# scrose/SVDSolver

Hardware: AMD Instinct MI355X
Metric: GFLOP/s for two-stage bidiag reduction, N×N fp64, 1/2/4/8 MI355X (higher is better)
Workload: dtype f64; 1 GPU; stream of independent two-stage bidiagonal reductions 8192x8192 f64, band 32, stage 2 = reference window geometry (compat); n=8192, band=32, global_batch=10, parallelism=replicas1, pipeline=stage 2 of matrix i on a second HIP stream beside stage 1 of matrix i+1, stage2_cus=32, lanes=10, stage2_streams=5, hw_queues=19

## Files before the change

svdsolver_amd/csrc/brd_blk.h:

```cpp
#pragma once

#include "brd_internal.h"

#include <hip/hip_ext.h>

#include <climits>

namespace brd {
namespace blk {

template <typename T> struct Mf;
template <> struct Mf<double> {
    typedef double v4 __attribute__((ext_vector_type(4)));
    static __device__ __forceinline__ v4 mma(double a, double b, v4 c) {
        return __builtin_amdgcn_mfma_f64_16x16x4f64(a, b, c, 0, 0, 0);
    }
    static __device__ __forceinline__ int crow(int q, int g) { return q + 4 * g; }
};
template <> struct Mf<float> {
    typedef float v4 __attribute__((ext_vector_type(4)));
    static __device__ __forceinline__ v4 mma(float a, float b, v4 c) {
        return __builtin_amdgcn_mfma_f32_16x16x4f32(a, b, c, 0, 0, 0);
    }
    static __device__ __forceinline__ int crow(int q, int g) { return 4 * q + g; }
// ... 11 lines not shown
constexpr int kWM = 64;
constexpr int kMT = 256;
#ifndef BRD_BLK_KSU
#define BRD_BLK_KSU 8
#endif
constexpr int kSU = BRD_BLK_KSU;

constexpr int kRpLds = 8192;
struct RpArgs {
    const void *src;  long ld;
    const void *vsrc; long vld;
    const void *bsrc; long bld;
    int K, M;
    int mtiles, ksplit, kper;
    int tiles, ns, wst;
    int nvirt;
    void *part; long mp;
    void *vpart;
    void *vout;
    int *counter;
    int *err;
    int has_fin;
    int vfold = 0;
    int va = 0, vb = 0;
};

constexpr int kPT = 256;
constexpr int kPI = 32;

constexpr int kGramRec = 1040;
struct PrepArgs {
    void *A; long lda;
    void *Lw; void *RwT; long ldr;
    const void *part; long mp; int ksplit;
    const void *G;
    const void *Tm;
    void *Qp;
    long mq;
    int c;
    int j;
    int items;
    int reduce, factor;
    const double *sgn;
    int split;
    long cc;
    int zfill;
// ... 286 lines not shown
template <typename T, int AUX = 0> __device__ __forceinline__ T buf_ld(__amdgpu_buffer_rsrc_t r, unsigned off) {
    if constexpr (sizeof(T) == 8)
        return __builtin_bit_cast(double, __builtin_amdgcn_raw_buffer_load_b64(r, (int)off, 0, AUX));
    else
        return __builtin_bit_cast(float, __builtin_amdgcn_raw_buffer_load_b32(r, (int)off, 0, AUX));
}
template <typename T, int AUX = 0> __device__ __forceinline__ void buf_st(T v, __amdgpu_buffer_rsrc_t r, unsigned off) {
    if constexpr (sizeof(T) == 8)
        __builtin_amdgcn_raw_buffer_store_b64(__builtin_bit_cast(u32x2_t, v), r, (int)off, 0, AUX);
    else
        __builtin_amdgcn_raw_buffer_store_b32(__builtin_bit_cast(unsigned, v), r, (int)off, 0, AUX);
}

template <typename F, typename... Args>
static inline void blk_launch(const char *kind, double flops, double bytes, F kernel, dim3 grid, dim3 block,
                              hipStream_t s, Args... args) {
    hipEvent_t ea, eb;
    if (api_prof_launch_events(kind, flops, bytes, &ea, &eb, (int)(grid.x * grid.y)))
        hipExtLaunchKernelGGL(kernel, grid, block, 0, s, ea, eb, 0, args...);
    else
        hipLaunchKernelGGL(kernel, grid, block, 0, s, args...);
}

bool rpass_dma_ok(bool yp, int K, int M, size_t elem, const void *src, long ld, const void *vsrc, long vld,
                  const void *bsrc, long bld);
int rpass_stage_k(size_t elem);
template <typename T>
void launch_k_rpass(bool yp, dim3 grid, const RpArgs &a, const FinArgs &f, hipStream_t s, double fl, double by);
template <typename T>
void launch_k_vsum(const T *vpart, T *vout, int nvirt, T *pbase, long pstride, const double *sgn, hipStream_t s);
template <typename T>
void launch_k_prep(bool lq, dim3 grid, const PrepArgs &p, hipStream_t s);
enum CqrKernel { kCqrGram, kCqrQ1, kCqrV, kCqrVInline, kCqrMid };
template <typename T>
void launch_k_cqr(CqrKernel which, int nwg, const CqrArgs &a, const FinArgs &f, hipStream_t s);
template <typename T>
void launch_k_blkupd(dim3 grid, const GemmArgs &g, hipStream_t s, double fl, double by);
template <typename T>
void launch_dist_unpack_v(const T *src, T *dst, int M, hipStream_t s);
template <typename T>
void launch_dist_psum(const T *part, int ks, long mp, int rows, T *buf, hipStream_t s);

}
}
```

svdsolver_amd/csrc/brd_blk_prep.hip:

```cpp
#include "brd_blk.h"

#include <climits>
#include <cstdlib>

namespace brd {
namespace blk {


#ifndef BRD_GRAM_LSCOPE
#define BRD_GRAM_LSCOPE __HIP_MEMORY_SCOPE_AGENT
#endif
#ifndef BRD_GRAM_SSCOPE
#define BRD_GRAM_SSCOPE __HIP_MEMORY_SCOPE_AGENT
#endif
template <typename FILL>
__device__ __forceinline__ void prep_gram(const PrepArgs &a, int nwv, int wv, int ipw, double *tile, double *red,
                                          double *smax, int *sflag, FILL &&fill) {
    typedef Mf<double>::v4 v4d;
    const int lane = threadIdx.x & 63, q = lane >> 4, l15 = lane & 15;
    const int nt = 64 * nwv, tl = 64 * wv + lane;
    __syncthreads();
    double *tw = tile + wv * 16 * 33;
    fill(tw);
    __builtin_amdgcn_fence(__ATOMIC_RELEASE, "wavefront");
// ... 498 lines not shown
    __builtin_amdgcn_fence(__ATOMIC_ACQUIRE, "wavefront");
    T *QpT = (T *)a.Qp;
    const bool vs = i0 + l15 < a.items;
#pragma unroll
    for (int it = 0; it < 8; ++it) {
        const int t = 4 * it + q;
        if (vs) QpT[(size_t)t * a.mq + i0 + l15] = Tb[w][l15 * 34 + t];
    }
    if (a.gram) {
        __shared__ double smax[4];
        __shared__ int sflag;
        double *st = reinterpret_cast<double *>(Gs);
        prep_gram(a, a.split ? 2 : 4, w, a.split ? kPI : 2 * kPI, st, st + 4 * 16 * 33, smax, &sflag,
                  [&](double *tw) {
                      for (int e = lane; e < 512; e += 64) {
                          const int i = e >> 5, t = e & 31;
                          tw[i * 33 + t] = i0 + i < a.items ? (double)Tb[w][i * 34 + t] : 0.0;
                      }
                  });
    }
}

template <typename T>
void launch_k_prep(bool lq, dim3 grid, const PrepArgs &p, hipStream_t s) {
    static_assert(NBMAX == 4, "the specialised panel indices below");
    const char *ge = getenv("BRD_PREP_GENERIC");
    const int jsel = (ge && atoi(ge) != 0) ? -100 : p.j;
    if (lq) {
        switch (jsel) {
        case 0: blk_launch("s1_prep", 0.0, 0.0, k_prep_lq<T, 0>, grid, dim3(kPT), s, p); return;
        case 1: blk_launch("s1_prep", 0.0, 0.0, k_prep_lq<T, 1>, grid, dim3(kPT), s, p); return;
        case 2: blk_launch("s1_prep", 0.0, 0.0, k_prep_lq<T, 2>, grid, dim3(kPT), s, p); return;
        case 3: blk_launch("s1_prep", 0.0, 0.0, k_prep_lq<T, 3>, grid, dim3(kPT), s, p); return;
        default: blk_launch("s1_prep", 0.0, 0.0, k_prep_lq<T, -1>, grid, dim3(kPT), s, p); return;
        }
    }
    switch (jsel == -100 ? -100 : (p.factor ? p.j : -p.j)) {
    case 1: blk_launch("s1_prep", 0.0, 0.0, k_prep_qr<T, 1, 1>, grid, dim3(kPT), s, p); return;
    case 2: blk_launch("s1_prep", 0.0, 0.0, k_prep_qr<T, 2, 1>, grid, dim3(kPT), s, p); return;
    case 3: blk_launch("s1_prep", 0.0, 0.0, k_prep_qr<T, 3, 1>, grid, dim3(kPT), s, p); return;
    case -4: blk_launch("s1_prep", 0.0, 0.0, k_prep_qr<T, 4, 0>, grid, dim3(kPT), s, p); return;
    default: blk_launch("s1_prep", 0.0, 0.0, k_prep_qr<T, -1, -1>, grid, dim3(kPT), s, p); return;
    }
}
template void launch_k_prep<double>(bool, dim3, const PrepArgs &, hipStream_t);
template void launch_k_prep<float>(bool, dim3, const PrepArgs &, hipStream_t);

}
}
```

svdsolver_amd/csrc/brd_blk_rpass.hip:

```cpp
#include "brd_blk.h"

#include <cstdlib>

namespace brd {
namespace blk {

template <typename T, bool YP, typename FA>
__global__ void __launch_bounds__(kRT, 1) k_rpass(RpArgs a, FA fin) {
    typedef typename G2<T>::v2 v2;
    typedef typename Mf<T>::v4 v4;
    const int tid = threadIdx.x, lane = tid & 63, w = (tid >> 6) & 3, kh = tid >> 8;
    const int q = lane >> 4, l15 = lane & 15;
    __shared__ __attribute__((aligned(16))) double rp_lds[kRpLds];
    if (a.has_fin && blockIdx.x == 0) {
        cqr_finish_entry<T>(fin, tid, rp_lds);
        return;
    }
    const int bid = blockIdx.x - a.has_fin;
    const bool virt = bid < a.nvirt;
    int mx, ks;
    if (virt) { mx = 0; ks = bid; }
    else      { const int r = bid - a.nvirt; mx = r % a.mtiles; ks = r / a.mtiles; }
    const T *S;
    long ld;
// ... 133 lines not shown
__global__ void __launch_bounds__(256) k_vsum(const T *vpart, T *vout, int nvirt, T *pbase, long pstride,
                                              const double *sgn) {
    const int e = blockIdx.x * 256 + threadIdx.x;
    if (blockIdx.x == 0 && threadIdx.x < 32 && pbase)
        pbase[(size_t)threadIdx.x * pstride] = (T)((double)pbase[(size_t)threadIdx.x * pstride] - sgn[threadIdx.x]);
    T v[32];
#pragma unroll
    for (int k = 0; k < 32; ++k) v[k] = vpart[(size_t)min(k, nvirt - 1) * 32 * kMT + e];
    T s = v[0];
#pragma unroll
    for (int k = 1; k < 32; ++k)
        if (k < nvirt) s += v[k];
    vout[e] = s;
}

#ifndef BRD_RPASS_HOIST
#define BRD_RPASS_HOIST 0
#endif
constexpr int kRS = 4;
template <int Y> __device__ __forceinline__ void rp_wait(bool five) {
    if (five) asm volatile("s_waitcnt vmcnt(%0)" ::"n"(5 * Y) : "memory");
    else      asm volatile("s_waitcnt vmcnt(%0)" ::"n"(4 * Y) : "memory");
}
constexpr int kSY = 272;
struct RpLdsD {
    double s[kRS][16 * kSY];
    double b[kRS][16 * 32];
};
template <typename T> constexpr int rp_epv() { return 16 / (int)sizeof(T); }
template <typename T> constexpr int rp_krk() { return 128 / (int)sizeof(T); }
template <typename T> __device__ __forceinline__ int rp_bswz(int k) {
    return sizeof(T) == 8 ? (k & 1) << 3 : ((k >> 1) & 1) << 2;
}

template <typename T, bool YP>
__global__ void __launch_bounds__(kRT, 1) k_rpass_d(RpArgs a, FinArgs fin) {
    static_assert(sizeof(FinLds) <= sizeof(RpLdsD), "cqr_finish's LDS");
    typedef typename Mf<T>::v4 v4;
    constexpr int E = sizeof(T), EPV = rp_epv<T>(), KRK = rp_krk<T>();
    constexpr int BVR = 32 / EPV;
    constexpr int BRI = 64 / BVR;
    __shared__ RpLdsD L;
    const int tid = threadIdx.x, lane = tid & 63, w = __builtin_amdgcn_readfirstlane(tid >> 6);
    const int q = lane >> 4, l15 = lane & 15;
    if (a.has_fin && blockIdx.x == 0) {
        cqr_finish_entry<T>(fin, tid, &L);
        return;
    }
    const int g = blockIdx.x - a.has_fin;
    const int tot = a.tiles * a.ns;
    const int uend = min(tot, (g + 1) * a.wst);
    constexpr unsigned kOut = 0x80000000u;
    const unsigned lds_s = (unsigned)(uintptr_t)&L.s[0][0], lds_b = (unsigned)(uintptr_t)&L.b[0][0];
    const T *B = (const T *)a.bsrc;
    const int mb = 32 * w;
    for (int u = g * a.wst; u < uend;) {
        const int tt = u / a.ns, segend = min(uend, (tt + 1) * a.ns);
        const bool virt = a.nvirt > 0 && tt == 0;
// ... 20 lines not shown
                const int i = 4 * w + uu, m = 8 * i + (lane >> 3), sl = lane & 7, pr = sl ^ ((m >> 1) & 7);
                const unsigned off = (m < M && k0 + EPV * pr < ke0) ? (unsigned)((m * (int)ld + EPV * pr) * E) : kOut;
                dma16(rs, off, 0, lds_s + (unsigned)(buf * sizeof(L.s[0]) + i * 1024));
            }
        };
        auto issue_b = [&](int st) {
            const int k0 = kb0 + KRK * st, buf = st % kRS;
            const u32x4_t rb = rsrc_of(B + (long)k0 * a.bld);
            const int kr = BRI * w + lane / BVR, sl = lane % BVR, tp = sl ^ rp_bswz<T>(kr);
            const unsigned off = k0 + kr < ke0 ? (unsigned)((kr * (int)a.bld + EPV * tp) * E) : kOut;
            dma16(rb, off, 0, lds_b + (unsigned)(buf * sizeof(L.b[0]) + w * 1024));
        };
        auto issue = [&](int st) {
#pragma unroll
            for (int uu = 0; uu < 4; ++uu) issue_src(st, uu);
            if (w < 4) issue_b(st);
        };

        v4 acc[2][2];
#pragma unroll
        for (int i = 0; i < 2; ++i)
#pragma unroll
            for (int j = 0; j < 2; ++j) acc[i][j] = v4{(T)0, (T)0, (T)0, (T)0};
#pragma unroll
        for (int st = 0; st < kRS - 1; ++st)
            if (st < nst) issue(st);
        for (int st = 0; st < nst; ++st) {
            const int younger = min(nst - 1 - st, kRS - 2);
            static_assert(kRS >= 2 && kRS <= 5, "rp_wait cases");
            if (kRS >= 5 && younger >= 3) rp_wait<3>(w < 4);
            else if (kRS >= 4 && younger >= 2) rp_wait<2>(w < 4);
            else if (kRS >= 3 && younger >= 1) rp_wait<1>(w < 4);
            else rp_wait<0>(w < 4);
            __syncthreads();
            if (st + kRS - 1 < nst) issue(st + kRS - 1);
            const int buf = st % kRS;
            const T *ls = (const T *)L.s[buf], *lb = (const T *)L.b[buf];
            constexpr int NS4 = KRK / 4;
            constexpr int HG = BRD_RPASS_HOIST ? NS4 : 1;
#pragma unroll
            for (int s0 = 0; s0 < NS4; s0 += HG) {
                T bt[HG][2], sm[HG][2];
#pragma unroll
                for (int u = 0; u < HG; ++u) {
                    const int k = 4 * (s0 + u) + q;
#pragma unroll
                    for (int h = 0; h < 2; ++h) {
                        const int t = 16 * h + l15;
                        bt[u][h] = lb[k * 32 + EPV * ((t / EPV) ^ rp_bswz<T>(k)) + t % EPV];
                    }
#pragma unroll
                    for (int p = 0; p < 2; ++p) {
                        const int m = mb + 16 * p + l15;
                        if constexpr (YP) sm[u][p] = ls[k * kSY + m];
                        else sm[u][p] = ls[m * KRK + EPV * ((k / EPV) ^ ((m >> 1) & 7)) + k % EPV];
                    }
                }
                if constexpr (BRD_RPASS_HOIST) __builtin_amdgcn_sched_barrier(0);
#pragma unroll
                for (int u = 0; u < HG; ++u)
#pragma unroll
                    for (int i = 0; i < 2; ++i)
#pragma unroll
                        for (int j = 0; j < 2; ++j) {
                            if constexpr (YP) acc[i][j] = Mf<T>::mma(bt[u][i], sm[u][j], acc[i][j]);
                            else acc[i][j] = Mf<T>::mma(sm[u][i], bt[u][j], acc[i][j]);
                        }
            }
        }
        T *out;
        long mp, sstride;
        if (virt) { out = (T *)a.vpart; mp = kMT; sstride = 32L * kMT; }
        else      { out = (T *)a.part + (size_t)mx * kMT * (YP ? 1 : 32); mp = a.mp; sstride = 32L * a.mp; }
        T *o = out + (size_t)slot * sstride;
        const bool vf = virt && a.vfold;
#pragma unroll
        for (int i = 0; i < 2; ++i)
#pragma unroll
            for (int j = 0; j < 2; ++j)
#pragma unroll
                for (int gg = 0; gg < 4; ++gg) {
                    const int r = Mf<T>::crow(q, gg);
                    size_t idx;
                    bool ok;
                    if (YP) { const int t = 16 * i + r, m = mb + 16 * j + l15; idx = (size_t)t * mp + m; ok = m < M; }
                    else    { const int m = mb + 16 * i + r, t = 16 * j + l15; idx = (size_t)m * 32 + t; ok = m < M; }
                    if (ok) {
                        if (vf) __hip_atomic_store(o + idx, acc[i][j][gg], __ATOMIC_RELAXED, __HIP_MEMORY_SCOPE_AGENT);
                        else    o[idx] = acc[i][j][gg];
                    }
                }
// ... 65 lines not shown
            }
        }
        u = segend;
        __syncthreads();
    }
}

static bool rpass_dma_enabled() {
    const char *e = getenv("BRD_RPASS_DMA");
    return !e || atoi(e) != 0;
}

bool rpass_dma_ok(bool yp, int K, int M, size_t elem, const void *src, long ld, const void *vsrc, long vld,
                  const void *bsrc, long bld) {
    const long epv = 16 / (long)elem;
    auto al = [&](const void *p, long l) { return p == nullptr || ((uintptr_t)p % 16 == 0 && l % epv == 0); };
    return rpass_dma_enabled() && (yp ? M % epv == 0 : K % epv == 0) && al(src, ld) && al(vsrc, vld) && al(bsrc, bld);
}
int rpass_stage_k(size_t elem) { return 128 / (int)elem; }

template <typename T>
void launch_k_rpass(bool yp, dim3 grid, const RpArgs &a, const FinArgs &f, hipStream_t s, double fl, double by) {
    if (a.wst > 0) {
        if (yp) blk_launch("s1_rpass", fl, by, k_rpass_d<T, true>, grid, dim3(kRT), s, a, f);
        else    blk_launch("s1_rpass", fl, by, k_rpass_d<T, false>, grid, dim3(kRT), s, a, f);
        return;
    }
    if (yp) blk_launch("s1_rpass", fl, by, k_rpass<T, true, FinArgs>, grid, dim3(kRT), s, a, f);
    else    blk_launch("s1_rpass", fl, by, k_rpass<T, false, FinArgs>, grid, dim3(kRT), s, a, f);
}
template <typename T>
void launch_k_vsum(const T *vpart, T *vout, int nvirt, T *pbase, long pstride, const double *sgn, hipStream_t s) {
    blk_launch("s1_prep", 0.0, 0.0, k_vsum<T>, dim3(32 * kMT / 256), dim3(256), s, vpart, vout, nvirt, pbase, pstride,
               sgn);
}
template void launch_k_rpass<double>(bool, dim3, const RpArgs &, const FinArgs &, hipStream_t, double, double);
template void launch_k_rpass<float>(bool, dim3, const RpArgs &, const FinArgs &, hipStream_t, double, double);
template void launch_k_vsum<double>(const double *, double *, int, double *, long, const double *, hipStream_t);
template void launch_k_vsum<float>(const float *, float *, int, float *, long, const double *, hipStream_t);

}
}
```

svdsolver_amd/csrc/brd_blk_upd.hip:

```cpp
#include "brd_blk.h"

#include <algorithm>
#include <cstdlib>

namespace brd {
namespace blk {

template <typename T>
struct GemmLds {
    T a[2][kGKC * kGM];
    T b[2][kGKC * kGBP];
};

template <typename T>
__global__ void __launch_bounds__(kGT, 2) k_blkupd(GemmArgs a) {
    typedef typename G2<T>::v2 v2;
    typedef typename Mf<T>::v4 v4;
    __shared__ GemmLds<T> L;
    const int tid = threadIdx.x, lane = tid & 63, w = tid >> 6;
    const int q = lane >> 4, l15 = lane & 15;
    const int tr = blockIdx.x / a.tiles_c, tc = blockIdx.x % a.tiles_c;
    const int r0 = tr * kGM, c0 = tc * kGM;
    const int wr = (w >> 1) * 64, wc = (w & 1) * 64;
    T *C = (T *)a.C;
// ... 337 lines not shown
        for (int c = 0; c < nc; ++c) {
            if (c + 1 < nc) asm volatile("s_waitcnt vmcnt(3)" ::: "memory");
            else            asm volatile("s_waitcnt vmcnt(0)" ::: "memory");
            __syncthreads();
            if (c + 2 < nc) issue_h(c + 2, (c + 2) % 3);
            chunk_mma_h(c % 3);
        }
        const Cio cc = cio_of(r0, c0, wrh);
#pragma unroll
        for (int i = 0; i < 2; ++i)
#pragma unroll
            for (int j = 0; j < 2; ++j)
#pragma unroll
                for (int g = 0; g < 4; ++g) cbuf[i][j][g] = buf_ld<T>(cc.r, c_at(cc, i, j, g));
#pragma unroll
        for (int i = 0; i < 2; ++i)
#pragma unroll
            for (int j = 0; j < 2; ++j)
#pragma unroll
                for (int g = 0; g < 4; ++g) buf_st<T>(cbuf[i][j][g] - acc[i][j][g], cc.r, c_at(cc, i, j, g));
    }
}

static int blkupd_persistent() {
    const char *e = getenv("BRD_BLKUPD_P");
    return e ? atoi(e) : 1;
}

template <typename T>
void launch_k_blkupd(dim3 grid, const GemmArgs &g, hipStream_t s, double fl, double by) {
    {
        const bool al = sizeof(T) == 8 || (g.ldr % 4 == 0 && (uintptr_t)g.RwT % 16 == 0 && (uintptr_t)g.Lw % 16 == 0);
        if (blkupd_persistent() && al) {
            static int cus = 0;
            if (!cus) {
                int dev = 0;
                hipGetDevice(&dev);
                hipDeviceGetAttribute(&cus, hipDeviceAttributeMultiprocessorCount, dev);
            }
            const int tgt = api_overlap_active() ? api_apply_target() : cus;
            GemmArgs gs = g;
            const char *he = getenv("BRD_BLKUPD_HALF");
            const int r = g.ntiles % tgt;
            gs.nh = 0;
            if ((he ? atoi(he) : 1) && r > 0 && 2 * r <= tgt) {
                gs.nfull = g.ntiles - r;
                gs.nh = 2 * r;
            }
            const int items = gs.nh > 0 ? gs.nfull + gs.nh : g.ntiles;
            const int grid = std::min<int>(items, tgt);
            if (gs.nh == 0) gs.nfull = g.ntiles;
            const char *xe = getenv("BRD_BLKUPD_XCD");
            const int tiles_r = g.ntiles / g.tiles_c;
            gs.xsr = gs.xsc = 0;
            if ((xe ? atoi(xe) : 0) && grid % 32 == 0 && gs.nfull >= grid && tiles_r >= 4 && g.tiles_c >= grid / 32) {
                gs.xsr = 4;
                gs.xsc = grid / 32;
            }
            blk_launch("s1_blkupd", fl, by, k_blkupd_p<T>, dim3(grid), dim3(kGT2), s, gs);
            return;
        }
    }
    blk_launch("s1_blkupd", fl, by, k_blkupd<T>, grid, dim3(kGT), s, g);
}
template void launch_k_blkupd<double>(dim3, const GemmArgs &, hipStream_t, double, double);
template void launch_k_blkupd<float>(dim3, const GemmArgs &, hipStream_t, double, double);

}
}
```

svdsolver_amd/csrc/brd_stage1_blk.hip:

```cpp
#include "brd.h"
#include "brd_blk.h"

#include <algorithm>
#include <cstdio>
#include <cstdlib>
#include <vector>

namespace brd {

using namespace blk;

struct BlkLayout {
    size_t lw, rwt, ub, part, vpart, vout, qp, tf, cws, ctr, sg, gpp, total;
    long ldr, mp;
    int ksmax, cwg;
};

static BlkLayout blk_layout(int m, int n, size_t elem) {
    BlkLayout L;
    L.ldr = (n + 1) & ~1L;
    L.mp = (std::max(m, n) + 1) & ~1L;
    L.ksmax = 32;
    L.cwg = kCW;
    size_t off = 0;
// ... 7 lines not shown
    L.qp = take((size_t)32 * L.mp * elem);
    L.tf = take((size_t)8 * 1024 * elem);
    L.cws = take(cqr_ws_doubles() * sizeof(double));
    L.ctr = take((64 + kCW) * sizeof(int));
    L.sg = take((size_t)(2 * NBMAX + 1) * 32 * sizeof(double));
    L.gpp = take((size_t)((std::max(m, n) + kPI - 1) / kPI) * kGramRec * sizeof(double));
    L.total = off;
    return L;
}

size_t blk_ws_bytes(int m, int n, size_t elem) { return blk_layout(m, n, elem).total; }

int blk_columns(int m, int n, int b) {
    if (b != 32 || m > kCW * kCT || n > kCW * kCT) return 0;
    int k0 = 0;
    while (n - k0 >= (NBMAX + 1) * 32) k0 += NBMAX * 32;
    return k0;
}

static constexpr int kLeanMaxN = 12288;
struct S1Launch {
    int target;
    bool lean;
};
static S1Launch s1_launch(int m, int n, int target) {
    return S1Launch{target, api_overlap_active() && std::max(m, n) <= kLeanMaxN};
}
static dim3 prep_grid(PrepArgs &p, const S1Launch &lc) {
    const int items = std::max(p.items, p.zfill);
    const int n1 = (items + kPI - 1) / kPI;
    const int mode = getenv("BRD_PREP_SPLIT") ? atoi(getenv("BRD_PREP_SPLIT")) : -1;
    p.split = mode == 0 ? 0 : (mode == 1 || (n1 <= lc.target && !lc.lean)) ? 1 : 0;
    return dim3(std::max(1, p.split ? n1 : (items + 2 * kPI - 1) / (2 * kPI)));
}

template <typename T>
static hipError_t launch_rpass(bool yp, const T *src, long ld, int K, int M, const T *bsrc, long bld, const T *vsrc,
                               long vld, char *ws, const BlkLayout &Ly, int *counter, int *err, hipStream_t s,
                               const S1Launch &lc, int *ksplit_out, const FinArgs *fin, T *pbase, long pstride,
                               const double *psgn, void *vout = nullptr, bool *vfolded = nullptr, int va = 0,
                               int vb = 0) {
    RpArgs a;
    a.src = src; a.ld = ld; a.vsrc = vsrc; a.vld = vld; a.bsrc = bsrc; a.bld = bld;
    a.K = K; a.M = M;
    a.mtiles = (M + kMT - 1) / kMT;
    static const double rpx = getenv("BRD_BLK_RPX") ? std::max(0.125, atof(getenv("BRD_BLK_RPX"))) : 1.0;
    int target = lc.lean ? std::max(1, lc.target / 2) : lc.target;
    target = std::max(1, (int)(target * rpx));
    int ks, nwg;
    a.tiles = a.ns = a.wst = 0;
    if (rpass_dma_ok(yp, K, M, sizeof(T), src, ld, vsrc, vld, bsrc, bld) && K > 0) {
        a.tiles = a.mtiles + (vsrc ? 1 : 0);
        const int krk = rpass_stage_k(sizeof(T));
        a.ns = (K + krk - 1) / krk;
// ... 6 lines not shown
        ks = 1;
        for (int t = 0; t < a.tiles; ++t)
            ks = std::max(ks, (int)(((long)(t + 1) * a.ns - 1) / wst - ((long)t * a.ns) / wst + 1));
        a.kper = 0;
    } else {
        ks = std::max(1, target / std::max(1, a.mtiles + 1));
        ks = std::min(ks, std::max(1, K / 64));
        ks = std::min(ks, Ly.ksmax);
        a.kper = ((K + ks - 1) / ks + 7) / 8 * 8;
        ks = (K + a.kper - 1) / a.kper;
        nwg = (vsrc ? ks : 0) + a.mtiles * ks;
    }
    a.ksplit = ks;
    a.nvirt = vsrc ? ks : 0;
    a.part = ws + Ly.part; a.mp = Ly.mp;
    a.vpart = ws + Ly.vpart; a.vout = vout ? vout : ws + Ly.vout;
    a.counter = counter;
    a.err = err;
    a.has_fin = fin ? 1 : 0;
    const FinArgs fa = fin ? *fin : FinArgs{};
    *ksplit_out = ks;
    dim3 grid(a.has_fin + nwg);
    const double fl = 2.0 * 32 * K * M, by = (double)K * M * sizeof(T);
    const char *vfe = getenv("BRD_VSUM_FOLD");
    const bool want = vfe ? atoi(vfe) != 0 : api_overlap_active();
    a.vfold = (vfolded && want && a.wst > 0 && a.nvirt > 0) ? 1 : 0;
    a.va = va; a.vb = vb;
    if (vfolded) *vfolded = a.vfold != 0;
    launch_k_rpass<T>(yp, grid, a, fa, s, fl, by);
    if (a.nvirt > 0 && !a.vfold) launch_k_vsum<T>((const T *)a.vpart, (T *)a.vout, a.nvirt, pbase, pstride, psgn, s);
    return hipGetLastError();
}

template <typename T>
static hipError_t launch_cqr(const T *src, long si, long st, int M, T *vdst, long vsi, long vst, T *vdst2, long vsi2,
                             long vst2, T *tout, T *apan, long asi, long ast, char *ws, const BlkLayout &Ly, int *err,
                             hipStream_t s, bool inl, const FinArgs &fin, int azero = 1, double *qcopy = nullptr,
                             bool gram_done = false) {
    CqrArgs a;
    a.rec = nullptr; a.nrec = 1; a.rme = 0; a.rctr = nullptr;
    a.Mg = M; a.goff = 0; a.top = 1;
    a.src = src; a.si = si; a.st = st; a.M = M;
    a.vdst = vdst; a.vsi = vsi; a.vst = vst;
    a.vdst2 = vdst2; a.vsi2 = vsi2; a.vst2 = vst2;
    a.tout = tout; a.apan = apan; a.asi = asi; a.ast = ast;
    const int nwg = (M + kCT - 1) / kCT;
    if (nwg > Ly.cwg) return hipErrorInvalidValue;
    a.ws = (double *)(ws + Ly.cws);
    a.err = err;
    a.azero = azero;
// ... 41 lines not shown
        p.gcnt = ctr + 64;
    };
    for (int k0 = 0; k0 < kend; k0 += NBMAX * 32) {
        for (int j = 0; j < NBMAX; ++j) {
            const int c = k0 + 32 * j;
            const int mr = m - c;
            const int n2 = n - c - 32;
            T *Tj = tf + 1024 * j, *Sj = tf + 1024 * (NBMAX + j);
            const FinArgs fq = fin_of(sgq + 32 * j, Tj, A + (size_t)c * lda + c, lda, 1);
            if (j == 0) {
                e = launch_cqr<T>(A + (size_t)c * lda + c, lda, 1, mr, Lw + (size_t)c * 256, 256, 1, nullptr, 0, 0, Tj,
                                  A + (size_t)c * lda + c, lda, 1, ws, Ly, err, s, false, fq);
            } else {
                PrepArgs p;
                p.A = A; p.lda = lda; p.Lw = Lw; p.RwT = RwT; p.ldr = ldr;
                p.part = ws + Ly.part; p.mp = Ly.mp; p.ksplit = ks_x;
                p.G = ws + Ly.vout; p.Tm = tf + 1024 * (NBMAX + j - 1);
                p.Qp = ws + Ly.qp; p.mq = Ly.mp;
                p.c = c; p.j = j; p.items = mr; p.reduce = 1; p.factor = 1;
                p.sgn = sg_prev;
                p.cc = c; p.zfill = 0;
                p.upatch = x_patch ? 1 : 0;
                gram_into(p, fold_qr);
                launch_k_prep<T>(false, prep_grid(p, lc), p, s);
                e = hipGetLastError();
                if (e != hipSuccess) return e;
                e = launch_cqr<T>((const T *)(ws + Ly.qp), 1, Ly.mp, mr, Lw + (size_t)c * 256 + 32 * j, 256, 1, nullptr, 0, 0, Tj,
                                  A + (size_t)c * lda + c, lda, 1, ws, Ly, err, s, false, fq, 1, nullptr, fold_qr);
            }
            if (e != hipSuccess) return e;
            int ks_y = 1;
            bool yfold = false;
            e = launch_rpass<T>(true, A + (size_t)c * lda + c + 32, lda, mr, n2, Lw + (size_t)c * 256 + 32 * j, 256,
                                Lw + (size_t)c * 256, 256, ws, Ly, ctr + 16, err, s, lc, &ks_y, &fq,
                                Lw + (size_t)c * 256 + 32 * j, 257, sgq + 32 * j, nullptr, &yfold, 32 * j, 32 * j);
            if (e != hipSuccess) return e;
            {
                PrepArgs p;
                p.A = A; p.lda = lda; p.Lw = Lw; p.RwT = RwT; p.ldr = ldr;
                p.part = ws + Ly.part; p.mp = Ly.mp; p.ksplit = ks_y;
                p.G = ws + Ly.vout; p.Tm = Tj;
                p.Qp = ws + Ly.qp; p.mq = Ly.mp;
                p.c = c; p.j = j; p.items = n2; p.reduce = 0; p.factor = 0;
                p.sgn = sgq + 32 * j;
                p.cc = c + 32; p.zfill = 0;
                p.vpatch = yfold ? 1 : 0;
                gram_into(p, fold_lq);
                launch_k_prep<T>(true, prep_grid(p, lc), p, s);
                e = hipGetLastError();
                if (e != hipSuccess) return e;
            }
            const bool inl = j == NBMAX - 1;
            const FinArgs fl = fin_of(sgl + 32 * j, Sj, A + (size_t)c * lda + c + 32, 1, lda);
            e = launch_cqr<T>((const T *)(ws + Ly.qp), 1, Ly.mp, n2, RwT + (size_t)(128 + 32 * j) * ldr + c + 32, 1, ldr,
                              Ub + (size_t)(c + 32) * 32, 32, 1, Sj, A + (size_t)c * lda + c + 32, 1, lda, ws, Ly, err, s,
                              inl, fl, 1, nullptr, fold_lq);
            if (e != hipSuccess) return e;
            bool xfold = false;
            e = launch_rpass<T>(false, A + (size_t)(c + 32) * lda + c + 32, lda, n2, m - c - 32,
                                Ub + (size_t)(c + 32) * 32, 32, RwT + c + 32, ldr, ws, Ly, ctr + 16, err, s,
                                lc, &ks_x, inl ? nullptr : &fl,
                                inl ? nullptr : RwT + (size_t)(128 + 32 * j) * ldr + c + 32, ldr + 1, sgl + 32 * j,
                                nullptr, &xfold, 32 * (j + 1), 32 * j);
            x_patch = !inl && xfold;
            if (e != hipSuccess) return e;
            sg_prev = inl ? sg0 : sgl + 32 * j;
        }
        const int k1 = k0 + NBMAX * 32;
        {
            PrepArgs p;
            p.A = A; p.lda = lda; p.Lw = Lw; p.RwT = RwT; p.ldr = ldr;
            p.part = ws + Ly.part; p.mp = Ly.mp; p.ksplit = ks_x;
            p.G = ws + Ly.vout; p.Tm = tf + 1024 * (2 * NBMAX - 1);
            p.Qp = ws + Ly.qp; p.mq = Ly.mp;
            p.c = k1; p.j = NBMAX; p.items = m - k1; p.reduce = 1; p.factor = 0;
            p.sgn = sg_prev;
            p.cc = k1; p.zfill = 0;
            launch_k_prep<T>(false, prep_grid(p, lc), p, s);
            e = hipGetLastError();
            if (e != hipSuccess) return e;
        }
        {
            GemmArgs g;
            g.C = A + (size_t)k1 * lda + k1; g.ldc = lda;
            g.rows = m - k1; g.cols = n - k1;
            g.Lw = Lw + (size_t)k1 * 256; g.RwT = RwT + k1; g.ldr = ldr;
            g.K = 256;
            g.tiles_c = (g.cols + kGM - 1) / kGM;
            const int tiles_r = (g.rows + kGM - 1) / kGM;
            g.ntiles = tiles_r * g.tiles_c;
            const int grid = g.ntiles;
            const double el = (double)g.rows * g.cols;
            launch_k_blkupd<T>(dim3(grid), g, s, 2.0 * 256 * el, (2.0 * el + 256.0 * (g.rows + g.cols)) * sizeof(T));
            e = hipGetLastError();
            if (e != hipSuccess) return e;
        }
    }
    return hipSuccess;
}

template hipError_t blk_ge2band<double>(double *, int, int, long, void *, hipStream_t, int, int *);
template hipError_t blk_ge2band<float>(float *, int, int, long, void *, hipStream_t, int, int *);

namespace {
struct DistBlk {
    size_t bc, rec, ar, total;
};
DistBlk dist_blk_layout(int m, int n, int P, int rank, size_t elem) {
    const BlkLayout Ly = blk_layout(m, std::max(dist_local_cols(n, 32, P, rank), 1), elem);
    DistBlk D;
    size_t off = Ly.total;
    auto take = [&](size_t bytes) { size_t o = off; off += (bytes + 255) & ~(size_t)255; return o; };
    D.bc = take((size_t)m * 32 * elem + 1032 * sizeof(double));
    D.rec = take((size_t)3 * P * kCqrRec * sizeof(double));
    D.ar = take(((size_t)m * 32 + 256 * 32 + 1024) * elem);
    D.total = off;
// ... 61 lines not shown
        double *cw = (double *)(ws + Ly.cws);
        pa.gram = 1;
        pa.gpp = (double *)(ws + Ly.gpp);
        pa.gout = cw;
        pa.gew = cw + 3072 * kCW;
        pa.gcnt = ctr + 64;
    };
    const T *s_prev = nullptr;
    for (int k0 = 0; k0 < kend; k0 += NBMAX * 32) {
        for (int j = 0; j < NBMAX; ++j) {
            const int p = k0 / 32 + j, c = 32 * p, mr = m - c, mx = m - c - 32;
            const int o = p % P, o2 = (p + 1) % P;
            const bool own = me == o, own2 = me == o2;
            const long lco = (long)(p / P) * 32;
            const long lcs = (long)dist_panels_before(p + 1, P, me) * 32;
            const int nc = n_loc - (int)lcs;
            T *Tj = tf + 1024 * j, *Sj = tf + 1024 * (NBMAX + j);
            T *sj_ar = ar + (size_t)mx * 32 + 256 * 32;
            double *qt = (double *)((char *)bc + (size_t)mr * 32 * sizeof(T));
            const bool fold_qr = own && j > 0 && (foldm & 1);
            if (j > 0) {
                PrepArgs pa = prep(c, j, mr, 1, own ? 1 : 0, ar + 256 * 32, 0, 1, ar, s_prev, sg0, lco);
                if (fold_qr) gram_into(pa);
                launch_k_prep<T>(false, prep_grid(pa, lc), pa, s);
                BD_HIP(hipGetLastError());
            }
            const FinArgs fq{qt, qt + 1024, sgq + 32 * j, Tj, own ? (void *)(A + (size_t)c * lda + lco) : nullptr, lda, 1};
            if (own) {
                const T *src = j == 0 ? A + (size_t)c * lda + lco : (const T *)(ws + Ly.qp);
                const long si = j == 0 ? lda : 1, st = j == 0 ? 1 : Ly.mp;
                BD_HIP(launch_cqr<T>(src, si, st, mr, Lw + (size_t)c * 256 + 32 * j, 256, 1, bc, 32, 1, Tj,
                                     A + (size_t)c * lda + lco, lda, 1, ws, Ly, err, s, false, fq, 1, qt, fold_qr));
            }
            {
                BD_TRY(C.bcast(bc, (size_t)mr * 32 * sizeof(T) + 1025 * sizeof(double), o, s));
                if (!own) launch_dist_unpack_v<T>(bc, Lw + (size_t)c * 256 + 32 * j, mr, s);
            }
            int ks_y = 1;
            BD_HIP(launch_rpass<T>(true, A + (size_t)c * lda + lcs, lda, mr, nc, Lw + (size_t)c * 256 + 32 * j, 256,
                                   Lw + (size_t)c * 256, 256, ws, Ly, ctr + 16, err, s, lc, &ks_y, &fq,
                                   Lw + (size_t)c * 256 + 32 * j, 257, sgq + 32 * j));
            {
                PrepArgs pa = prep(c, j, nc, 0, 0, ws + Ly.part, Ly.mp, ks_y, ws + Ly.vout, Tj, sgq + 32 * j, lcs);
                launch_k_prep<T>(true, prep_grid(pa, lc), pa, s);
                BD_HIP(hipGetLastError());
            }
            {
                CqrArgs a;
                a.src = ws + Ly.qp; a.si = 1; a.st = Ly.mp; a.M = std::max(nc, 0);
                a.vdst = RwT + (size_t)(128 + 32 * j) * ldr + lcs; a.vsi = 1; a.vst = ldr;
                a.vdst2 = Ub + (size_t)lcs * 32; a.vsi2 = 32; a.vst2 = 1;
                a.tout = Sj;
                a.apan = A + (size_t)c * lda + lcs; a.asi = 1; a.ast = lda;
                a.ws = (double *)(ws + Ly.cws);
                a.err = err;
                a.azero = 1;
                a.qcopy = nullptr;
                a.rec = rec; a.nrec = P; a.rme = me; a.rctr = ctr + 40;
                a.Mg = n - c - 32;
                a.goff = (long)((me - o2 + P) % P) * kCW * kCT;
                a.top = own2 ? 1 : 0;
                const int nwg = std::max(1, (a.M + kCT - 1) / kCT);
                const FinArgs fl{cws + cqr_ws_qt(), cws + cqr_ws_zero(), sgl + 32 * j, own2 ? sj_ar : Sj,
                                 own2 ? (void *)(A + (size_t)c * lda + lcs) : nullptr, 1, lda};
                if (!own2) BD_HIP(hipMemsetAsync(sj_ar, 0, 1024 * sizeof(T), s));
                const size_t rb = (size_t)kCqrRec * sizeof(double);
                launch_k_cqr<T>(kCqrGram, nwg, a, fl, s);
                BD_TRY(C.allgather(rec + (size_t)me * kCqrRec, rec, rb, s));
                launch_k_cqr<T>(kCqrQ1, nwg, a, fl, s);
                BD_TRY(C.allgather(rec + (size_t)(P + me) * kCqrRec, rec + (size_t)P * kCqrRec, rb, s));
                launch_k_cqr<T>(kCqrMid, nwg, a, fl, s);
                BD_TRY(C.allgather(rec + (size_t)(2 * P + me) * kCqrRec, rec + (size_t)2 * P * kCqrRec, rb, s));
                launch_k_cqr<T>(own2 ? kCqrVInline : kCqrV, nwg, a, fl, s);
                BD_HIP(hipGetLastError());
            }
            if (nc > 0) {
                int ks_x = 1;
                BD_HIP(launch_rpass<T>(false, A + (size_t)(c + 32) * lda + lcs, lda, nc, mx, Ub + lcs * 32, 32,
                                       RwT + lcs, ldr, ws, Ly, ctr + 16, err, s, lc, &ks_x, nullptr, nullptr, 0,
                                       nullptr, ar));
                launch_dist_psum<T>((const T *)(ws + Ly.part), ks_x, Ly.mp, mx, ar + 256 * 32, s);
            } else {
                BD_HIP(hipMemsetAsync(ar, 0, ((size_t)mx * 32 + 256 * 32) * sizeof(T), s));
            }
            BD_TRY(C.allreduce_sum(ar, (size_t)mx * 32 + 256 * 32 + 1024, dt, s));
            s_prev = sj_ar;
        }
        const int k1 = k0 + NBMAX * 32;
        {
            PrepArgs pa = prep(k1, NBMAX, m - k1, 1, 0, ar + 256 * 32, 0, 1, ar, s_prev, sg0, 0);
            launch_k_prep<T>(false, prep_grid(pa, lc), pa, s);
            BD_HIP(hipGetLastError());
        }
        const long lck = (long)dist_panels_before(k1 / 32, P, me) * 32;
        const int cols = n_loc - (int)lck;
        if (cols > 0) {
            GemmArgs g;
            g.C = A + (size_t)k1 * lda + lck; g.ldc = lda;
            g.rows = m - k1; g.cols = cols;
            g.Lw = Lw + (size_t)k1 * 256; g.RwT = RwT + lck; g.ldr = ldr;
            g.K = 256;
            g.tiles_c = (g.cols + kGM - 1) / kGM;
            g.ntiles = ((g.rows + kGM - 1) / kGM) * g.tiles_c;
            const double el = (double)g.rows * g.cols;
            launch_k_blkupd<T>(dim3(g.ntiles), g, s, 2.0 * 256 * el, (2.0 * el + 256.0 * (g.rows + g.cols)) * sizeof(T));
            BD_HIP(hipGetLastError());
        }
    }
    return BRD_OK;
}
template int blk_ge2band_dist<double>(double *, int, int, long, Comm &, void *, hipStream_t, int, int *);
template int blk_ge2band_dist<float>(float *, int, int, long, Comm &, void *, hipStream_t, int, int *);

}
```

Baseline: 27810 GFLOP/s.

## Cache stage-1 env settings per call and add fast-issue and staggered rpass pipelines

Reads the stage-1 tuning environment variables once per reduction into an S1Env struct, so per-launch getenv calls go away. The DMA rpass kernel gains a precomputed-offset issue path (dma16x4 with incrementing pointers), which is on by default via BRD_RPASS_FASTISSUE. It also gains an optional staggered-wave pipeline, off unless BRD_RPASS_STAGGER is set. The fast-issue path uses inline asm that writes m0 and adds new template instantiations.

```diff
diff --git a/svdsolver_amd/csrc/brd_blk.h b/svdsolver_amd/csrc/brd_blk.h
--- a/svdsolver_amd/csrc/brd_blk.h
+++ b/svdsolver_amd/csrc/brd_blk.h
@@ -57,6 +57,7 @@
     int *err;
     int has_fin;
     int vfold = 0;
+    int stagger = 0;
     int va = 0, vb = 0;
 };
 
@@ -389,6 +390,16 @@
         hipLaunchKernelGGL(kernel, grid, block, 0, s, args...);
 }
 
+struct S1Env {
+    int prep_split;
+    int vsum_fold;
+    bool prep_generic;
+    bool blkupd_p;
+    bool blkupd_half;
+    bool blkupd_xcd;
+    bool rp_stagger;
+};
+
 bool rpass_dma_ok(bool yp, int K, int M, size_t elem, const void *src, long ld, const void *vsrc, long vld,
                   const void *bsrc, long bld);
 int rpass_stage_k(size_t elem);
@@ -397,12 +408,12 @@
 template <typename T>
 void launch_k_vsum(const T *vpart, T *vout, int nvirt, T *pbase, long pstride, const double *sgn, hipStream_t s);
 template <typename T>
-void launch_k_prep(bool lq, dim3 grid, const PrepArgs &p, hipStream_t s);
+void launch_k_prep(bool lq, dim3 grid, const PrepArgs &p, hipStream_t s, const S1Env &env);
 enum CqrKernel { kCqrGram, kCqrQ1, kCqrV, kCqrVInline, kCqrMid };
 template <typename T>
 void launch_k_cqr(CqrKernel which, int nwg, const CqrArgs &a, const FinArgs &f, hipStream_t s);
 template <typename T>
-void launch_k_blkupd(dim3 grid, const GemmArgs &g, hipStream_t s, double fl, double by);
+void launch_k_blkupd(dim3 grid, const GemmArgs &g, hipStream_t s, double fl, double by, const S1Env &env);
 template <typename T>
 void launch_dist_unpack_v(const T *src, T *dst, int M, hipStream_t s);
 template <typename T>
diff --git a/svdsolver_amd/csrc/brd_blk_prep.hip b/svdsolver_amd/csrc/brd_blk_prep.hip
--- a/svdsolver_amd/csrc/brd_blk_prep.hip
+++ b/svdsolver_amd/csrc/brd_blk_prep.hip
@@ -544,10 +544,9 @@
 }
 
 template <typename T>
-void launch_k_prep(bool lq, dim3 grid, const PrepArgs &p, hipStream_t s) {
+void launch_k_prep(bool lq, dim3 grid, const PrepArgs &p, hipStream_t s, const S1Env &env) {
     static_assert(NBMAX == 4, "the specialised panel indices below");
-    const char *ge = getenv("BRD_PREP_GENERIC");
-    const int jsel = (ge && atoi(ge) != 0) ? -100 : p.j;
+    const int jsel = env.prep_generic ? -100 : p.j;
     if (lq) {
         switch (jsel) {
         case 0: blk_launch("s1_prep", 0.0, 0.0, k_prep_lq<T, 0>, grid, dim3(kPT), s, p); return;
@@ -565,8 +564,8 @@
     default: blk_launch("s1_prep", 0.0, 0.0, k_prep_qr<T, -1, -1>, grid, dim3(kPT), s, p); return;
     }
 }
-template void launch_k_prep<double>(bool, dim3, const PrepArgs &, hipStream_t);
-template void launch_k_prep<float>(bool, dim3, const PrepArgs &, hipStream_t);
+template void launch_k_prep<double>(bool, dim3, const PrepArgs &, hipStream_t, const S1Env &);
+template void launch_k_prep<float>(bool, dim3, const PrepArgs &, hipStream_t, const S1Env &);
 
 }
 }
diff --git a/svdsolver_amd/csrc/brd_blk_rpass.hip b/svdsolver_amd/csrc/brd_blk_rpass.hip
--- a/svdsolver_amd/csrc/brd_blk_rpass.hip
+++ b/svdsolver_amd/csrc/brd_blk_rpass.hip
@@ -179,6 +179,37 @@
     if (five) asm volatile("s_waitcnt vmcnt(%0)" ::"n"(5 * Y) : "memory");
     else      asm volatile("s_waitcnt vmcnt(%0)" ::"n"(4 * Y) : "memory");
 }
+#ifndef BRD_RPASS_RD
+#define BRD_RPASS_RD (kRS - 1)
+#endif
+#ifndef BRD_RPASS_FASTISSUE
+#define BRD_RPASS_FASTISSUE 1
+#endif
+#ifndef BRD_RPASS_PRIO
+#define BRD_RPASS_PRIO 0
+#endif
+constexpr int kRD = BRD_RPASS_RD;
+static_assert(kRD >= 1 && kRD <= 3 && kRD <= kRS - 1, "rp_wait_n cases; a slot is re-issued only after its last read");
+__device__ __forceinline__ void rp_wait_n(int younger, bool five) {
+    if (younger >= 2) rp_wait<2>(five);
+    else if (younger == 1) rp_wait<1>(five);
+    else rp_wait<0>(five);
+}
+__device__ __forceinline__ void dma16x4(u32x4_t rsrc, const unsigned (&voff)[4], unsigned l0, unsigned l1, unsigned l2,
+                                        unsigned l3) {
+    unsigned keep;
+    asm volatile("s_mov_b32 %0, m0\n\t"
+                 "s_mov_b32 m0, %6\n\ts_nop 0\n\tbuffer_load_dwordx4 %1, %5, 0 offen lds\n\t"
+                 "s_mov_b32 m0, %7\n\ts_nop 0\n\tbuffer_load_dwordx4 %2, %5, 0 offen lds\n\t"
+                 "s_mov_b32 m0, %8\n\ts_nop 0\n\tbuffer_load_dwordx4 %3, %5, 0 offen lds\n\t"
+                 "s_mov_b32 m0, %9\n\ts_nop 0\n\tbuffer_load_dwordx4 %4, %5, 0 offen lds\n\t"
+                 "s_mov_b32 m0, %0"
+                 : "=&s"(keep)
+                 : "v"(voff[0]), "v"(voff[1]), "v"(voff[2]), "v"(voff[3]), "s"(rsrc),
+                   "s"(__builtin_amdgcn_readfirstlane(l0)), "s"(__builtin_amdgcn_readfirstlane(l1)),
+                   "s"(__builtin_amdgcn_readfirstlane(l2)), "s"(__builtin_amdgcn_readfirstlane(l3))
+                 : "memory");
+}
 constexpr int kSY = 272;
 struct RpLdsD {
     double s[kRS][16 * kSY];
@@ -190,7 +221,7 @@
     return sizeof(T) == 8 ? (k & 1) << 3 : ((k >> 1) & 1) << 2;
 }
 
-template <typename T, bool YP>
+template <typename T, bool YP, bool SG>
 __global__ void __launch_bounds__(kRT, 1) k_rpass_d(RpArgs a, FinArgs fin) {
     static_assert(sizeof(FinLds) <= sizeof(RpLdsD), "cqr_finish's LDS");
     typedef typename Mf<T>::v4 v4;
@@ -257,9 +288,100 @@
         for (int i = 0; i < 2; ++i)
 #pragma unroll
             for (int j = 0; j < 2; ++j) acc[i][j] = v4{(T)0, (T)0, (T)0, (T)0};
+        const bool five = w < 4;
+        unsigned voff[4], lof[4], voffb;
+#pragma unroll
+        for (int uu = 0; uu < 4; ++uu) {
+            const int i = 4 * w + uu;
+            if constexpr (YP) {
+                constexpr int IPR = 256 * E / 1024;
+                const int kr = i / IPR, h = i % IPR, m = (1024 * h + 16 * lane) / E;
+                voff[uu] = m < M ? (unsigned)((kr * (int)ld + m) * E) : kOut;
+                lof[uu] = (unsigned)((kr * kSY + 1024 / E * h) * E);
+            } else {
+                const int m = 8 * i + (lane >> 3), sl = lane & 7, pr = sl ^ ((m >> 1) & 7);
+                voff[uu] = m < M ? (unsigned)((m * (int)ld + EPV * pr) * E) : kOut;
+                lof[uu] = (unsigned)(i * 1024);
+            }
+        }
+        {
+            const int kr = BRI * w + lane / BVR, sl = lane % BVR, tp = sl ^ rp_bswz<T>(kr);
+            voffb = (unsigned)((kr * (int)a.bld + EPV * tp) * E);
+        }
+        const long sstep = (YP ? (long)KRK * ld : (long)KRK) * E, bstep = (long)KRK * a.bld * E;
+        const char *sp = (const char *)(S + (YP ? (long)kb0 * ld : (long)kb0));
+        const char *bp = (const char *)(B + (long)kb0 * a.bld);
+        const int nfull = (ke0 - kb0) / KRK;
+        int isst = 0, isbuf = 0;
+        auto issue_next = [&]() {
+            if (isst < nfull) {
+                const unsigned ls0 = lds_s + (unsigned)(isbuf * sizeof(L.s[0]));
+                dma16x4(rsrc_of(sp), voff, ls0 + lof[0], ls0 + lof[1], ls0 + lof[2], ls0 + lof[3]);
+                if (five) dma16(rsrc_of(bp), voffb, 0, lds_b + (unsigned)(isbuf * sizeof(L.b[0]) + w * 1024));
+            } else {
+                issue(isst);
+            }
+            ++isst;
+            isbuf = isbuf + 1 == kRS ? 0 : isbuf + 1;
+            sp += sstep;
+            bp += bstep;
+        };
+        if constexpr (SG) {
+            const bool late = w >= 4;
+            auto wait_next = [&](int st) {
+                if (st + 1 < nst) rp_wait_n(min(st + kRD, nst - 1) - (st + 1), five);
+            };
+#pragma unroll
+            for (int st = 0; st < kRD; ++st)
+                if (st < nst) issue_next();
+            rp_wait_n(min(nst, kRD) - 1, five);
+            __builtin_amdgcn_s_barrier();
+            if (late) __builtin_amdgcn_s_barrier();
+            constexpr int NS4 = KRK / 4;
+            int buf = 0;
+            for (int st = 0; st < nst; ++st) {
+                const T *ls = (const T *)L.s[buf], *lb = (const T *)L.b[buf];
+                buf = buf + 1 == kRS ? 0 : buf + 1;
+                T bt[NS4][2], sm[NS4][2];
+#pragma unroll
+                for (int u = 0; u < NS4; ++u) {
+                    const int k = 4 * u + q;
+#pragma unroll
+                    for (int h = 0; h < 2; ++h) {
+                        const int t = 16 * h + l15;
+                        bt[u][h] = lb[k * 32 + EPV * ((t / EPV) ^ rp_bswz<T>(k)) + t % EPV];
+                    }
+#pragma unroll
+                    for (int p = 0; p < 2; ++p) {
+                        const int m = mb + 16 * p + l15;
+                        if constexpr (YP) sm[u][p] = ls[k * kSY + m];
+                        else sm[u][p] = ls[m * KRK + EPV * ((k / EPV) ^ ((m >> 1) & 7)) + k % EPV];
+                    }
+                }
+                if (st + kRD < nst) issue_next();
+                if (late) wait_next(st);
+                __builtin_amdgcn_sched_barrier(0);
+                lds_barrier();
+                __builtin_amdgcn_sched_barrier(0);
+                if constexpr (BRD_RPASS_PRIO) __builtin_amdgcn_s_setprio(1);
+#pragma unroll
+                for (int u = 0; u < NS4; ++u)
+#pragma unroll
+                    for (int i = 0; i < 2; ++i)
+#pragma unroll
+                        for (int j = 0; j < 2; ++j) {
+                            if constexpr (YP) acc[i][j] = Mf<T>::mma(bt[u][i], sm[u][j], acc[i][j]);
+                            else acc[i][j] = Mf<T>::mma(sm[u][i], bt[u][j], acc[i][j]);
+                        }
+                if constexpr (BRD_RPASS_PRIO) __builtin_amdgcn_s_setprio(0);
+                __builtin_amdgcn_sched_barrier(0);
+                if (!late) wait_next(st);
+                if (!(late && st == nst - 1)) __builtin_amdgcn_s_barrier();
+            }
+        } else {
 #pragma unroll
         for (int st = 0; st < kRS - 1; ++st)
-            if (st < nst) issue(st);
+            if (st < nst) { if constexpr (BRD_RPASS_FASTISSUE) issue_next(); else issue(st); }
         for (int st = 0; st < nst; ++st) {
             const int younger = min(nst - 1 - st, kRS - 2);
             static_assert(kRS >= 2 && kRS <= 5, "rp_wait cases");
@@ -268,7 +390,7 @@
             else if (kRS >= 3 && younger >= 1) rp_wait<1>(w < 4);
             else rp_wait<0>(w < 4);
             __syncthreads();
-            if (st + kRS - 1 < nst) issue(st + kRS - 1);
+            if (st + kRS - 1 < nst) { if constexpr (BRD_RPASS_FASTISSUE) issue_next(); else issue(st + kRS - 1); }
             const int buf = st % kRS;
             const T *ls = (const T *)L.s[buf], *lb = (const T *)L.b[buf];
             constexpr int NS4 = KRK / 4;
@@ -302,6 +424,7 @@
                             else acc[i][j] = Mf<T>::mma(sm[u][i], bt[u][j], acc[i][j]);
                         }
             }
+        }
         }
         T *out;
         long mp, sstride;
@@ -413,8 +536,13 @@
 template <typename T>
 void launch_k_rpass(bool yp, dim3 grid, const RpArgs &a, const FinArgs &f, hipStream_t s, double fl, double by) {
     if (a.wst > 0) {
-        if (yp) blk_launch("s1_rpass", fl, by, k_rpass_d<T, true>, grid, dim3(kRT), s, a, f);
-        else    blk_launch("s1_rpass", fl, by, k_rpass_d<T, false>, grid, dim3(kRT), s, a, f);
+        if (a.stagger) {
+            if (yp) blk_launch("s1_rpass", fl, by, k_rpass_d<T, true, true>, grid, dim3(kRT), s, a, f);
+            else    blk_launch("s1_rpass", fl, by, k_rpass_d<T, false, true>, grid, dim3(kRT), s, a, f);
+        } else {
+            if (yp) blk_launch("s1_rpass", fl, by, k_rpass_d<T, true, false>, grid, dim3(kRT), s, a, f);
+            else    blk_launch("s1_rpass", fl, by, k_rpass_d<T, false, false>, grid, dim3(kRT), s, a, f);
+        }
         return;
     }
     if (yp) blk_launch("s1_rpass", fl, by, k_rpass<T, true, FinArgs>, grid, dim3(kRT), s, a, f);
diff --git a/svdsolver_amd/csrc/brd_blk_upd.hip b/svdsolver_amd/csrc/brd_blk_upd.hip
--- a/svdsolver_amd/csrc/brd_blk_upd.hip
+++ b/svdsolver_amd/csrc/brd_blk_upd.hip
@@ -383,16 +383,11 @@
     }
 }
 
-static int blkupd_persistent() {
-    const char *e = getenv("BRD_BLKUPD_P");
-    return e ? atoi(e) : 1;
-}
-
 template <typename T>
-void launch_k_blkupd(dim3 grid, const GemmArgs &g, hipStream_t s, double fl, double by) {
+void launch_k_blkupd(dim3 grid, const GemmArgs &g, hipStream_t s, double fl, double by, const S1Env &env) {
     {
         const bool al = sizeof(T) == 8 || (g.ldr % 4 == 0 && (uintptr_t)g.RwT % 16 == 0 && (uintptr_t)g.Lw % 16 == 0);
-        if (blkupd_persistent() && al) {
+        if (env.blkupd_p && al) {
             static int cus = 0;
             if (!cus) {
                 int dev = 0;
@@ -401,20 +396,18 @@
             }
             const int tgt = api_overlap_active() ? api_apply_target() : cus;
             GemmArgs gs = g;
-            const char *he = getenv("BRD_BLKUPD_HALF");
             const int r = g.ntiles % tgt;
             gs.nh = 0;
-            if ((he ? atoi(he) : 1) && r > 0 && 2 * r <= tgt) {
+            if (env.blkupd_half && r > 0 && 2 * r <= tgt) {
                 gs.nfull = g.ntiles - r;
                 gs.nh = 2 * r;
             }
             const int items = gs.nh > 0 ? gs.nfull + gs.nh : g.ntiles;
             const int grid = std::min<int>(items, tgt);
             if (gs.nh == 0) gs.nfull = g.ntiles;
-            const char *xe = getenv("BRD_BLKUPD_XCD");
             const int tiles_r = g.ntiles / g.tiles_c;
             gs.xsr = gs.xsc = 0;
-            if ((xe ? atoi(xe) : 0) && grid % 32 == 0 && gs.nfull >= grid && tiles_r >= 4 && g.tiles_c >= grid / 32) {
+            if (env.blkupd_xcd && grid % 32 == 0 && gs.nfull >= grid && tiles_r >= 4 && g.tiles_c >= grid / 32) {
                 gs.xsr = 4;
                 gs.xsc = grid / 32;
             }
@@ -424,8 +417,8 @@
     }
     blk_launch("s1_blkupd", fl, by, k_blkupd<T>, grid, dim3(kGT), s, g);
 }
-template void launch_k_blkupd<double>(dim3, const GemmArgs &, hipStream_t, double, double);
-template void launch_k_blkupd<float>(dim3, const GemmArgs &, hipStream_t, double, double);
-
-}
-}
+template void launch_k_blkupd<double>(dim3, const GemmArgs &, hipStream_t, double, double, const S1Env &);
+template void launch_k_blkupd<float>(dim3, const GemmArgs &, hipStream_t, double, double, const S1Env &);
+
+}
+}
diff --git a/svdsolver_amd/csrc/brd_stage1_blk.hip b/svdsolver_amd/csrc/brd_stage1_blk.hip
--- a/svdsolver_amd/csrc/brd_stage1_blk.hip
+++ b/svdsolver_amd/csrc/brd_stage1_blk.hip
@@ -53,14 +53,30 @@
 struct S1Launch {
     int target;
     bool lean;
+    S1Env env;
 };
+static S1Env s1_env() {
+    auto num = [](const char *name, int unset) {
+        const char *e = getenv(name);
+        return e ? atoi(e) : unset;
+    };
+    S1Env v;
+    v.prep_split = num("BRD_PREP_SPLIT", -1);
+    v.vsum_fold = getenv("BRD_VSUM_FOLD") ? (num("BRD_VSUM_FOLD", 0) != 0 ? 1 : 0) : -1;
+    v.prep_generic = num("BRD_PREP_GENERIC", 0) != 0;
+    v.blkupd_p = num("BRD_BLKUPD_P", 1) != 0;
+    v.blkupd_half = num("BRD_BLKUPD_HALF", 1) != 0;
+    v.blkupd_xcd = num("BRD_BLKUPD_XCD", 0) != 0;
+    v.rp_stagger = num("BRD_RPASS_STAGGER", 0) != 0;
+    return v;
+}
 static S1Launch s1_launch(int m, int n, int target) {
-    return S1Launch{target, api_overlap_active() && std::max(m, n) <= kLeanMaxN};
+    return S1Launch{target, api_overlap_active() && std::max(m, n) <= kLeanMaxN, s1_env()};
 }
 static dim3 prep_grid(PrepArgs &p, const S1Launch &lc) {
     const int items = std::max(p.items, p.zfill);
     const int n1 = (items + kPI - 1) / kPI;
-    const int mode = getenv("BRD_PREP_SPLIT") ? atoi(getenv("BRD_PREP_SPLIT")) : -1;
+    const int mode = lc.env.prep_split;
     p.split = mode == 0 ? 0 : (mode == 1 || (n1 <= lc.target && !lc.lean)) ? 1 : 0;
     return dim3(std::max(1, p.split ? n1 : (items + 2 * kPI - 1) / (2 * kPI)));
 }
@@ -113,10 +129,10 @@
     *ksplit_out = ks;
     dim3 grid(a.has_fin + nwg);
     const double fl = 2.0 * 32 * K * M, by = (double)K * M * sizeof(T);
-    const char *vfe = getenv("BRD_VSUM_FOLD");
-    const bool want = vfe ? atoi(vfe) != 0 : api_overlap_active();
+    const bool want = lc.env.vsum_fold >= 0 ? lc.env.vsum_fold != 0 : api_overlap_active();
     a.vfold = (vfolded && want && a.wst > 0 && a.nvirt > 0) ? 1 : 0;
     a.va = va; a.vb = vb;
+    a.stagger = lc.env.rp_stagger ? 1 : 0;
     if (vfolded) *vfolded = a.vfold != 0;
     launch_k_rpass<T>(yp, grid, a, fa, s, fl, by);
     if (a.nvirt > 0 && !a.vfold) launch_k_vsum<T>((const T *)a.vpart, (T *)a.vout, a.nvirt, pbase, pstride, psgn, s);
@@ -204,7 +220,7 @@
                 p.cc = c; p.zfill = 0;
                 p.upatch = x_patch ? 1 : 0;
                 gram_into(p, fold_qr);
-                launch_k_prep<T>(false, prep_grid(p, lc), p, s);
+                launch_k_prep<T>(false, prep_grid(p, lc), p, s, lc.env);
                 e = hipGetLastError();
                 if (e != hipSuccess) return e;
                 e = launch_cqr<T>((const T *)(ws + Ly.qp), 1, Ly.mp, mr, Lw + (size_t)c * 256 + 32 * j, 256, 1, nullptr, 0, 0, Tj,
@@ -228,7 +244,7 @@
                 p.cc = c + 32; p.zfill = 0;
                 p.vpatch = yfold ? 1 : 0;
                 gram_into(p, fold_lq);
-                launch_k_prep<T>(true, prep_grid(p, lc), p, s);
+                launch_k_prep<T>(true, prep_grid(p, lc), p, s, lc.env);
                 e = hipGetLastError();
                 if (e != hipSuccess) return e;
             }
@@ -258,7 +274,7 @@
             p.c = k1; p.j = NBMAX; p.items = m - k1; p.reduce = 1; p.factor = 0;
             p.sgn = sg_prev;
             p.cc = k1; p.zfill = 0;
-            launch_k_prep<T>(false, prep_grid(p, lc), p, s);
+            launch_k_prep<T>(false, prep_grid(p, lc), p, s, lc.env);
             e = hipGetLastError();
             if (e != hipSuccess) return e;
         }
@@ -273,7 +289,7 @@
             g.ntiles = tiles_r * g.tiles_c;
             const int grid = g.ntiles;
             const double el = (double)g.rows * g.cols;
-            launch_k_blkupd<T>(dim3(grid), g, s, 2.0 * 256 * el, (2.0 * el + 256.0 * (g.rows + g.cols)) * sizeof(T));
+            launch_k_blkupd<T>(dim3(grid), g, s, 2.0 * 256 * el, (2.0 * el + 256.0 * (g.rows + g.cols)) * sizeof(T), lc.env);
             e = hipGetLastError();
             if (e != hipSuccess) return e;
         }
@@ -381,7 +397,7 @@
             if (j > 0) {
                 PrepArgs pa = prep(c, j, mr, 1, own ? 1 : 0, ar + 256 * 32, 0, 1, ar, s_prev, sg0, lco);
                 if (fold_qr) gram_into(pa);
-                launch_k_prep<T>(false, prep_grid(pa, lc), pa, s);
+                launch_k_prep<T>(false, prep_grid(pa, lc), pa, s, lc.env);
                 BD_HIP(hipGetLastError());
             }
             const FinArgs fq{qt, qt + 1024, sgq + 32 * j, Tj, own ? (void *)(A + (size_t)c * lda + lco) : nullptr, lda, 1};
@@ -401,7 +417,7 @@
                                    Lw + (size_t)c * 256 + 32 * j, 257, sgq + 32 * j));
             {
                 PrepArgs pa = prep(c, j, nc, 0, 0, ws + Ly.part, Ly.mp, ks_y, ws + Ly.vout, Tj, sgq + 32 * j, lcs);
-                launch_k_prep<T>(true, prep_grid(pa, lc), pa, s);
+                launch_k_prep<T>(true, prep_grid(pa, lc), pa, s, lc.env);
                 BD_HIP(hipGetLastError());
             }
             {
@@ -448,7 +464,7 @@
         const int k1 = k0 + NBMAX * 32;
         {
             PrepArgs pa = prep(k1, NBMAX, m - k1, 1, 0, ar + 256 * 32, 0, 1, ar, s_prev, sg0, 0);
-            launch_k_prep<T>(false, prep_grid(pa, lc), pa, s);
+            launch_k_prep<T>(false, prep_grid(pa, lc), pa, s, lc.env);
             BD_HIP(hipGetLastError());
         }
         const long lck = (long)dist_panels_before(k1 / 32, P, me) * 32;
@@ -462,7 +478,7 @@
             g.tiles_c = (g.cols + kGM - 1) / kGM;
             g.ntiles = ((g.rows + kGM - 1) / kGM) * g.tiles_c;
             const double el = (double)g.rows * g.cols;
-            launch_k_blkupd<T>(dim3(g.ntiles), g, s, 2.0 * 256 * el, (2.0 * el + 256.0 * (g.rows + g.cols)) * sizeof(T));
+            launch_k_blkupd<T>(dim3(g.ntiles), g, s, 2.0 * 256 * el, (2.0 * el + 256.0 * (g.rows + g.cols)) * sizeof(T), lc.env);
             BD_HIP(hipGetLastError());
         }
     }
```

Result: no change. 28000 GFLOP/s, median of 6 (+0.7%).
